# pfnet/pfrl

Hardware: AMD Instinct MI355X
Metric: env-steps/sec whole node (DQN 256 envs sharded over the GPUs) (higher is better)
Workload: dtype f32

## Files before the change

### include/pfrl_amd.h

```cpp
#ifndef PFRL_AMD_H
#define PFRL_AMD_H

#include <stdint.h>

#ifdef __cplusplus
extern "C" {
#endif

#define PFRL_TAG_ABSENT 0
#define PFRL_TAG_PY 1
#define PFRL_TAG_F32 2
#define PFRL_TAG_F64 3

#define PFRL_MAX_LEVELS 40
#define PFRL_MAX_NSTEP 16
#define PFRL_MAX_STACK 8

#define PFRL_OPT_MAX_TENSORS 24

#define PFRL_POW_CORRECTLY_ROUNDED 0
#define PFRL_POW_GLIBC 1
#define PFRL_POW_GLIBC_FMA 2
#define PFRL_ERR_ARG (-2)

// ... 241 lines not shown
                           float *g_sigma_b, int64_t out_features, int64_t in_features,
                           void *stream);

int pfrl_conv2d_nhwc_fwd(const float *x, const float *w, const float *bias, float *y, int32_t N,
                         int32_t H, int32_t W, int32_t C, int32_t Cout, int32_t R, int32_t S,
                         int32_t stride, int32_t relu, int32_t planar_out, int32_t splits,
                         void *stream);
int pfrl_conv2d_nhwc_bwd_data(const float *dy, const float *dy_mask, const float *w,
                              const float *a_prev, float *dx, int32_t N, int32_t H, int32_t W,
                              int32_t C, int32_t Cout, int32_t R, int32_t S, int32_t stride,
                              int32_t perm_p, int32_t perm_c, void *stream);
int pfrl_conv2d_nhwc_bwd_weight(const float *dy, const float *dy_mask, const float *x, float *dw_part,
                                float *db_part, int64_t dw_stride, int64_t db_stride, int32_t N,
                                int32_t H, int32_t W, int32_t C, int32_t Cout, int32_t R, int32_t S,
                                int32_t stride, int32_t splits, void *stream);
int pfrl_conv2d_u8nhwc4_fwd(const uint8_t *x, float divisor, const float *w, const float *bias,
                            float *y, int32_t N, int32_t H, int32_t W, int32_t Cout, int32_t R,
                            int32_t S, int32_t stride, int32_t relu, int32_t planar_out, void *stream);
int pfrl_conv2d_u8nhwc4_bwd_weight(const float *dy, const float *dy_mask, const uint8_t *x,
                                   float divisor, float *dw_part, float *db_part, int64_t dw_stride,
                                   int64_t db_stride, int32_t N, int32_t H, int32_t W, int32_t Cout,
                                   int32_t R, int32_t S, int32_t stride, int32_t splits, void *stream);
int pfrl_conv2d_nhwc_bwd_weight_ride(
    const float *dy, const float *dy_mask, const float *x, float *dw_part, float *db_part,
    int64_t dw_stride, int64_t db_stride, int32_t N, int32_t H, int32_t W, int32_t C, int32_t Cout,
    int32_t R, int32_t S, int32_t stride, int32_t splits, int32_t n_ride, float *const *ride_param,
    const float *const *ride_grad, float *const *ride_square_avg, float *const *ride_grad_avg,
    const int64_t *ride_numel, float lr, float alpha, float eps, float weight_decay, int centered,
    void *stream);
int pfrl_conv2d_nhwc_bwd(const float *dy, const float *dy_mask, const float *w, const float *a_prev,
                         const float *x, float *dx, float *dw_part, float *db_part, int64_t dw_stride,
                         int64_t db_stride, int32_t N, int32_t H, int32_t W, int32_t C, int32_t Cout,
                         int32_t R, int32_t S, int32_t stride, int32_t perm_p, int32_t perm_c,
                         int32_t splits, void *stream);
int pfrl_splitk_reduce(int32_t n_tasks, const float *const *host_part, float *const *host_out,
                       const float *const *host_bias, const int64_t *host_stride,
                       const int32_t *host_n, const int32_t *host_splits, const int32_t *host_ncol,
                       const int32_t *host_relu, void *stream);
int pfrl_clip_grad_norm(int32_t n_tensors, float *const *grads, const int64_t *numel, float max_norm,
                        double *partial_ws, float *out_norm_coef, void *stream);
int pfrl_splitk_group(const float *part, int64_t stride, int32_t n, int32_t splits, int32_t groups,
                      float *out, int64_t out_stride, void *stream);
int pfrl_linear_fwd(const float *x, const float *w, const float *bias, float *y, int32_t M, int32_t K,
                    int32_t N, int32_t relu, int32_t splits, void *stream);
int pfrl_linear_bwd_weight(const float *dy, const float *dy_mask, const float *x, float *dw_part,
                           float *db_part, int64_t dw_stride, int64_t db_stride, int32_t M, int32_t K,
                           int32_t N, int32_t splits, void *stream);
int pfrl_linear_small_fwd(const float *x, const float *w, const float *bias, float *y, int32_t M,
                          int32_t K, int32_t N, void *stream);
int pfrl_dqn_act_head(const float *h, const float *w, const float *bias, const int32_t *choice,
                      float *q, int64_t *greedy, int64_t *action, int32_t M, int32_t K, int32_t N,
                      void *stream);
int pfrl_qnet_plan_images(int32_t images);
int pfrl_linear_small_bwd(const float *dy, const float *x, const float *w, float *dx, float *dw,
                          float *db, int32_t M, int32_t K, int32_t N, void *stream);

int pfrl_linear_fwd_twin(const float *const *x, const float *const *x2, int32_t K1,
                         const float *const *w, const float *const *bias, float *const *y, int32_t M,
                         int32_t K, int32_t N, int32_t relu, void *stream);
int pfrl_linear_bwd_twin(const float *const *dy, const float *const *dy_mask, const float *const *w,
                         const float *const *x, const float *const *x2, int32_t K1, float *const *dx,
                         float *const *dw_part,
                         float *const *db_part, int64_t dw_stride, int64_t db_stride, int32_t M,
                         int32_t K, int32_t N, int32_t splits, void *stream);
int pfrl_linear_small_fwd_twin(const float *const *x, const float *const *w, const float *const *bias,
                               float *const *y, int32_t M, int32_t K, int32_t N, void *stream);
int pfrl_linear_small_bwd_twin(const float *const *dy, const float *const *x, const float *const *w,
                               float *const *dx, float *const *dw, float *const *db, int32_t M,
                               int32_t K, int32_t N, void *stream);
int pfrl_twin_input_grad(const float *const *dy, const float *const *dy_mask, const float *const *w,
                         int32_t ldw, int32_t col0, int32_t ncol, float *dx, int32_t M, int32_t N,
                         void *stream);

int pfrl_squashed_gaussian_fwd(const float *loc, int64_t ld_loc, const float *scale, int64_t ld_scale,
                               const float *eps, float *action, float *logp, float *neg_logp, int32_t B,
                               int32_t A, void *stream);
int pfrl_squashed_gaussian_bwd(const float *g_action, const float *g_logp, const float *action,
                               const float *eps, const float *scale, int64_t ld_scale, float *g_loc,
                               float *g_scale, int32_t B, int32_t A, void *stream);
int pfrl_squashed_head_fwd(const float *x, int64_t ldx, float clamp_lo, float clamp_hi, int32_t mode,
                           const float *eps, float *action, float *logp, float *neg_logp, int32_t B,
                           int32_t A, void *stream);
int pfrl_squashed_head_bwd(const float *g_action, const float *g_logp, const float *action,
                           const float *eps, const float *x, int64_t ldx, float clamp_lo, float clamp_hi,
                           int32_t mode, float *g_x, int32_t B, int32_t A, void *stream);
int pfrl_soft_update(int32_t n_tensors, float *const *dst, const float *const *src,
                     const int64_t *numel, double tau, void *stream);
int pfrl_adam_step(int32_t n_tensors, float *const *params, const float *const *grads,
                   float *const *exp_avg, float *const *exp_avg_sq, float *const *steps,
                   const int64_t *numel, double lr, double beta1, double beta2, double eps,
                   double weight_decay, void *ticket, void *stream);
int pfrl_adam_step_ex(int32_t n_tensors, float *const *params, const float *const *grads,
                      const int64_t *slab_stride, const int32_t *n_slabs, float *const *exp_avg,
                      float *const *exp_avg_sq, float *const *steps, float *const *soft_dst, double tau,
                      const int64_t *numel, double lr, double beta1, double beta2, double eps,
                      double weight_decay, void *ticket, void *stream);
int pfrl_sac_temperature_loss(const float *log_temperature, const float *log_prob,
                              float entropy_target, float *loss, int32_t B, void *stream);
int pfrl_sac_temperature_step(float *log_temperature, const float *log_prob, float entropy_target,
                              float *loss, float *exp_avg, float *exp_avg_sq, float *step, double lr,
                              double beta1, double beta2, double eps, double weight_decay, int32_t B,
                              void *stream);
int pfrl_sac_target_q(const float *reward, const float *discount, const float *terminal,
                      const float *next_q1, const float *next_q2, const float *next_log_prob,
                      const float *log_temperature, float temperature, float *target_q, int32_t B,
                      void *stream);
// ... 86 lines not shown
```

### pfrl_amd/_native.py

```python
import ctypes
import os
import shutil
import subprocess

_HERE = os.path.dirname(os.path.abspath(__file__))
CSRC = os.path.join(_HERE, "csrc")
LIB_DIR = os.path.join(_HERE, "lib")
LIB_PATH = os.path.join(LIB_DIR, "libpfrl_amd.so")
_LIB_OVERRIDE = os.environ.get("PFRL_AMD_LIB")
SOURCES = ["frames.hip", "replay.hip", "sumtree.hip", "rollout.hip", "optim.hip", "tdloss.hip", "bias_act.hip", "noisy.hip", "c51.hip", "dueling.hip", "qnet.hip", "actor.hip", "hostplan.hip", "philox.hip", "ppo_gaussian.hip", "trpo.hip"]
HIPCC_FLAGS = [
    "--offload-arch=gfx950", "-O3", "-std=c++17", "-fPIC",
    "-ffp-contract=off", "-fno-fast-math",
    "-mllvm", "-amdgpu-kernarg-preload-count=16",
    "-mllvm", "-amdgpu-mfma-vgpr-form",
]

MAX_LEVELS = 40
MAX_NSTEP = 16
MAX_STACK = 8


def _hipcc():
    for cand in (shutil.which("hipcc"), "/opt/rocm/bin/hipcc"):
# ... 123 lines not shown
    "pfrl_tree_update_errors_write_sample": (ctypes.c_int, "Rqppifdifdddiiqppppqpppppppppidqpp"),
    "pfrl_tree_sample": (ctypes.c_int, "Rqpppppppppidqpp"),
    "pfrl_tree_update_errors_f32": (ctypes.c_int, "Rqppifdifdddiip"),
    "pfrl_tree_update_errors_write_f32": (ctypes.c_int, "Rqppifdifdddiiqppppp"),
    "pfrl_h2d_async": (ctypes.c_int, "ppqp"),
    "pfrl_powf_host": (ctypes.c_int, "ipfpq"),
    "pfrl_powf_host_variant": (ctypes.c_int, "fq"),
    "pfrl_powf_device": (ctypes.c_int, "ipfpqp"),
    "pfrl_tree_set_priorities": (ctypes.c_int, "Rqpppip"),
    "pfrl_gae_scan": (ctypes.c_int, "qqpppppddippp"),
    "pfrl_a2c_returns": (ctypes.c_int, "qqppppddip"),
    "pfrl_adv_stats": (ctypes.c_int, "pqppp"),
    "pfrl_ppo_minibatch": (ctypes.c_int, "qpppipppppippppppp"),
    "pfrl_ppo_act_head": (ctypes.c_int, "pppppppppppiiipp"),
    "pfrl_ppo_loss": (ctypes.c_int, "pppppppiiffffppppp"),
    "pfrl_ppo_head_loss": (ctypes.c_int, "ppppppppppiiiffffppippp"),
    "pfrl_ppo_gaussian_act": (ctypes.c_int, "pppppppiip"),
    "pfrl_ppo_gaussian_loss": (ctypes.c_int, "ppppppppiiffffpppppp"),
    "pfrl_ppo_minibatch_f32act": (ctypes.c_int, "qpppippppipippppppp"),
    "pfrl_trpo_gaussian_eval": (ctypes.c_int, "pppppppiifppppp"),
    "pfrl_cg_workgroup_reach": (ctypes.c_int, []),
    "pfrl_cg_init": (ctypes.c_int, "ppppppqp"),
    "pfrl_cg_step": (ctypes.c_int, "ppppppqfp"),
    "pfrl_trpo_scale_step": (ctypes.c_int, "ppdpppqp"),
    "pfrl_params_axpy": (ctypes.c_int, "ippppfp"),
    "pfrl_rmsprop_step": (ctypes.c_int, "ipppppffffip"),
    "pfrl_rmsprop_fused_step": (ctypes.c_int, "ipffffip"),
    "pfrl_dqn_td_loss": (ctypes.c_int, "ppppppppqiiippppp"),
    "pfrl_dqn_head_td_loss": (ctypes.c_int, "ppppppppppiiiiipppppiqpppfp"),
    "pfrl_bias_relu_fwd": (ctypes.c_int, "pppqiqp"),
    "pfrl_bias_relu_bwd": (ctypes.c_int, "ppppppqiiqp"),
    "pfrl_c51_loss": (ctypes.c_int, "pppppppppiiiippppp"),
    "pfrl_dueling_softmax_fwd": (ctypes.c_int, "pppqiip"),
    "pfrl_dueling_softmax_bwd": (ctypes.c_int, "ppppqiip"),
    "pfrl_noisy_weights_fwd": (ctypes.c_int, "pppppppqqp"),
    "pfrl_noisy_weights_bwd": (ctypes.c_int, "pppppqqp"),
    "pfrl_conv2d_nhwc_fwd": (ctypes.c_int, "ppppiiiiiiiiiiip"),
    "pfrl_conv2d_nhwc_bwd_data": (ctypes.c_int, "pppppiiiiiiiiiip"),
    "pfrl_conv2d_nhwc_bwd_weight": (ctypes.c_int, "pppppqqiiiiiiiiip"),
    "pfrl_conv2d_nhwc_bwd_weight_ride": (ctypes.c_int, "pppppqqiiiiiiiiiipppppffffip"),
    "pfrl_conv2d_nhwc_bwd": (ctypes.c_int, "ppppppppqqiiiiiiiiiiip"),
    "pfrl_splitk_reduce": (ctypes.c_int, "ippppppppp"),
    "pfrl_splitk_reduce_noisy": (ctypes.c_int, "ippppppppppp"),
    "pfrl_splitk_group": (ctypes.c_int, "pqiiipqp"),
    "pfrl_clip_grad_norm": (ctypes.c_int, "ippfppp"),
    "pfrl_linear_noisy_fwd": (ctypes.c_int, "pppppppiiiiip"),
    "pfrl_linear_noisy_fwd_pair": (ctypes.c_int, "pippppppiipip"),
    "pfrl_linear_fwd": (ctypes.c_int, "ppppiiiiip"),
    "pfrl_linear_bwd_weight": (ctypes.c_int, "pppppqqiiiip"),
    "pfrl_linear_small_fwd": (ctypes.c_int, "ppppiiip"),
    "pfrl_linear_small_bwd": (ctypes.c_int, "ppppppiiip"),
    "pfrl_dqn_act_head": (ctypes.c_int, "pppppppiiip"),
    "pfrl_qnet_plan_images": (ctypes.c_int, "i"),
    "pfrl_squashed_gaussian_fwd": (ctypes.c_int, "pqpqppppiip"),
    "pfrl_squashed_gaussian_bwd": (ctypes.c_int, "pppppqppiip"),
    "pfrl_squashed_head_fwd": (ctypes.c_int, "pqffippppiip"),
    "pfrl_squashed_head_bwd": (ctypes.c_int, "pppppqffipiip"),
    "pfrl_soft_update": (ctypes.c_int, "ipppdp"),
    "pfrl_adam_step": (ctypes.c_int, "ippppppdddddpp"),
    "pfrl_adam_step_ex": (ctypes.c_int, "ippppppppdpdddddpp"),
    "pfrl_sac_temperature_loss": (ctypes.c_int, "ppfpip"),
    "pfrl_sac_temperature_step": (ctypes.c_int, "ppfppppdddddip"),
    "pfrl_sac_target_q": (ctypes.c_int, "pppppppfpip"),
    "pfrl_half_mse_fwd": (ctypes.c_int, "pppip"),
    "pfrl_half_mse_bwd": (ctypes.c_int, "ppppip"),
    "pfrl_half_mse_twin_fwd": (ctypes.c_int, "ppppip"),
    "pfrl_half_mse_twin_bwd": (ctypes.c_int, "ppppip"),
    "pfrl_linear_fwd_twin": (ctypes.c_int, "ppipppiiiip"),
    "pfrl_linear_bwd_twin": (ctypes.c_int, "pppppipppqqiiiip"),
    "pfrl_linear_small_fwd_twin": (ctypes.c_int, "ppppiiip"),
    "pfrl_linear_small_bwd_twin": (ctypes.c_int, "ppppppiiip"),
    "pfrl_twin_input_grad": (ctypes.c_int, "pppiiipiip"),
    "pfrl_sac_policy_loss_fwd": (ctypes.c_int, "ppppfppppip"),
    "pfrl_sac_policy_loss_bwd": (ctypes.c_int, "ppppfpppip"),
    "pfrl_philox_normal": (ctypes.c_int, "QQipppppip"),
    "pfrl_profile_enable": (ctypes.c_int, "i"),
    "pfrl_profile_collect": (ctypes.c_int64, "pppq"),
}

_CODES = {
    "p": ctypes.c_void_p, "q": ctypes.c_int64, "Q": ctypes.c_uint64, "i": ctypes.c_int,
    "f": ctypes.c_float, "d": ctypes.c_double,
    "T": ctypes.POINTER(TableDesc), "R": ctypes.POINTER(TreeDesc),
    "H": ctypes.POINTER(HostStoreDesc), "P": ctypes.c_void_p,
}

_lib = None


def lib():
    global _lib
    if _lib is not None:
        return _lib
    if not os.path.exists(LIB_PATH):
        raise RuntimeError(
            "pfrl_amd: %s is missing.  The device replay path has no CPU fallback; "
            "run `python -c 'import __graft_entry__ as g; g.build()'` (needs hipcc)." % LIB_PATH
        )
    L = ctypes.CDLL(_LIB_OVERRIDE or LIB_PATH)
    for name, (res, args) in EXPORTS.items():
        fn = getattr(L, name)
        fn.restype = res
        fn.argtypes = [_CODES[c] for c in args] if isinstance(args, str) else args
    _lib = L
    return L

# ... 52 lines not shown
```

### pfrl_amd/agents/dqn.py

```python
import collections
import copy
import os
from logging import getLogger

import numpy as np
import torch
import torch.nn.functional as F

from pfrl_amd import agent
from pfrl_amd.replay_buffer import (AbstractEpisodicReplayBuffer, DeviceExperienceBatch,
                                    ReplayUpdater, batch_experiences,
                                    batch_recurrent_experiences)
from pfrl_amd.utils.batch_states import batch_states
from pfrl_amd.utils.clip_l2_grad_norm import clip_l2_grad_norm_
from pfrl_amd.utils.contexts import evaluating
from pfrl_amd.utils.copy_param import synchronize_parameters
from pfrl_amd.utils.recurrent import (get_recurrent_state_at, mask_recurrent_state_at,
                                      one_step_forward, pack_and_forward,
                                      recurrent_state_as_numpy)


class _Pending:
    def __repr__(self):
        return "greedy(pending)"
# ... 98 lines not shown
        self.gamma = gamma
        self.explorer = explorer
        self.gpu = gpu
        self.target_update_interval = target_update_interval
        self.clip_delta = clip_delta
        self.phi = phi
        self.target_update_method = target_update_method
        self.soft_update_tau = soft_update_tau
        self.batch_accumulator = batch_accumulator
        assert batch_accumulator in ("mean", "sum")
        self.logger = logger
        self.batch_states = batch_states
        self.replay_updater = ReplayUpdater(
            replay_buffer=replay_buffer,
            update_func=self.update_from_episodes if self.recurrent else self.update,
            batchsize=minibatch_size,
            episodic_update=self.recurrent, episodic_update_len=episodic_update_len,
            n_times_update=n_times_update, replay_start_size=replay_start_size,
            update_interval=update_interval)
        self.minibatch_size = minibatch_size
        self.episodic_update_len = episodic_update_len
        self.replay_start_size = replay_start_size
        self.update_interval = update_interval
        self.max_grad_norm = max_grad_norm
        assert target_update_interval % update_interval == 0, \
            "target_update_interval should be a multiple of update_interval"
        self.t = 0
        self.optim_t = 0
        self._cumulative_steps = 0
        self.target_model = make_target_model_as_copy(self.model)
        self.q_record = _DeviceRecord(1000)
        self.loss_record = _DeviceRecord(100)
        self.batch_last_obs = []
        self.batch_last_action = []
        self.train_recurrent_states = None
        self.train_prev_recurrent_states = None
        self.test_recurrent_states = None
        if (self.replay_buffer.capacity is not None
                and self.replay_buffer.capacity < self.replay_updater.replay_start_size):
            raise ValueError("Replay start size cannot exceed replay buffer capacity.")
        from pfrl_amd.distributed import GradientAllReducer

        self.grad_reducer = GradientAllReducer(self.model)
        on_gpu = self.device.type == "cuda"
        self.use_graphs = on_gpu if use_graphs is None else bool(use_graphs and on_gpu)
        self.step_fused_gather = on_gpu if step_fused_gather is None else \
            bool(step_fused_gather and on_gpu)
        self.batch_target_pass = self.step_fused_gather if batch_target_pass is None else \
            bool(batch_target_pass and self.step_fused_gather)
        self.fused_td_loss = bool(fused_td_loss)
        self.step_fused_chunks = tuple(step_fused_chunks)
        self._chunks_set_by_caller = tuple(step_fused_chunks) != (0.1, 0.4)
        self._target_raw_bufs = {}
        self._single_bufs = {}
        self.range_graphs = os.environ.get("PFRL_RANGE_GRAPHS", "1") != "0"
        self.device_step = (on_gpu and self.step_fused_gather
                            and os.environ.get("PFRL_DEVICE_STEP", "1") != "0")
        self._last_actions_dev = None
        self._analytic_backward = None
        self._graphed = None
        self._last_y = None
        self._replay_stream = None
        self._fwd_event = None
        from pfrl_amd.replay_buffers.prioritized import PrioritizedReplayBuffer

        want_overlap = (self.use_graphs and isinstance(replay_buffer, PrioritizedReplayBuffer)
                        and getattr(replay_buffer, "is_device", False))
        if want_overlap if replay_overlap is None else (replay_overlap and want_overlap):
            self._replay_stream = torch.cuda.Stream(self.device)
            self._fwd_event = torch.cuda.Event()
            self._replay_stream.wait_stream(torch.cuda.current_stream(self.device))
            replay_buffer.set_replay_stream(self._replay_stream)

    @property
    def cumulative_steps(self):
        return self._cumulative_steps

    def sync_target_network(self):
        self._flush_backward()
        synchronize_parameters(src=self.model, dst=self.target_model,
                               method=self.target_update_method, tau=self.soft_update_tau)

    def update(self, experiences, errors_out=None, _gathered=None):
        self._flush_backward()
        if isinstance(experiences, DeviceExperienceBatch):
            has_weight = experiences.has_weight
        else:
            has_weight = "weight" in experiences[0][0]
        exp_batch = _gathered if _gathered is not None else batch_experiences(
            experiences, device=self.device, phi=self.phi, gamma=self.gamma,
            batch_states=self.batch_states)
        if self._replay_stream is not None and isinstance(experiences, DeviceExperienceBatch):
            if self._graphed is not None and self.use_graphs and has_weight:
                self._graphed.prefill(exp_batch, True)
            torch.cuda.current_stream(self.device).wait_event(experiences.store.ready_event)
        if has_weight and "weights" not in exp_batch:
            exp_batch["weights"] = torch.tensor([e[0]["weight"] for e in experiences],
                                                device=self.device, dtype=torch.float32)
        self._update_from_batch(exp_batch, has_weight, errors_out)

    def update_from_episodes(self, episodes, errors_out=None):
        assert errors_out is None, "Recurrent DQN does not support PrioritizedBuffer"
        episodes = sorted(episodes, key=len, reverse=True)
        exp_batch = batch_recurrent_experiences(episodes, device=self.device, phi=self.phi,
                                                gamma=self.gamma, batch_states=self.batch_states)
        self._update_from_batch(exp_batch)
# ... 35 lines not shown

    _late = None
    _in_train_step = False

    def _late_backward_ok(self):
        if self.__dict__.get("_late") is None:
            self._late = []
            self._late_enabled = os.environ.get("PFRL_LATE_BACKWARD", "1") != "0"
        return (self._late_enabled and self._in_train_step
                and not getattr(self._graphed, "split_for_allreduce", False))

    def _flush_backward(self):
        late = self.__dict__.get("_late")
        if late:
            pending = list(late)
            del late[:]
            for replay_rest in pending:
                replay_rest()

    def _graphed_step(self, exp_batch, want_errors, deferred=None, after_forward=None, late=None):
        if self._graphed is None:
            from pfrl_amd.agents.graphed_update import GraphedUpdate

            self._graphed = GraphedUpdate(self)
            self._graphed.pipeline = self._replay_stream is not None
        try:
            loss, delta, y = self._graphed.run(exp_batch, want_errors, after_forward, late)
        except Exception as e:
            if self._graphed.graphs:
                raise
            self.logger.warning("HIP-graph capture of the update failed (%s); running eagerly", e)
            self.use_graphs = False
            loss, delta = self._compute_loss(exp_batch, want_errors=want_errors)
            self.loss_record.extend(loss)
            self.optimizer.zero_grad()
            loss.backward()
            self.grad_reducer.all_reduce()
            if self.max_grad_norm is not None:
                clip_l2_grad_norm_(self.model.parameters(), self.max_grad_norm)
            self.optimizer.step()
            return loss, delta
        if deferred is not None:
            deferred.append((loss, y))
        else:
            self.loss_record.extend(loss.clone())
            self.q_record.extend(y.clone())
        return loss, delta

    def _target_is_deterministic(self):
        from pfrl_amd.nn.noisy_linear import FactorizedNoisyLinear

        return not any(isinstance(m, (FactorizedNoisyLinear, torch.nn.Dropout))
                       for m in self.target_model.modules())

    def _precompute_target_raw(self, next_states):
        with torch.no_grad():
            av = self.target_model(next_states)
        if hasattr(av, "q_dist"):
            self._target_z_values = av.z_values
            return av.q_dist
        return av.q_values

    def _action_value(self, model, states, recurrent_state):
        if self.recurrent:
            return pack_and_forward(model, states, recurrent_state)[0]
        return model(states)

    def _target_next_action_value(self, exp_batch):
        raw = exp_batch.get("target_next_raw")
        if raw is None:
            return self._action_value(self.target_model, exp_batch["next_state"],
                                      exp_batch.get("next_recurrent_state"))
        if raw.ndim == 3:
            from pfrl_amd.action_value import DistributionalDiscreteActionValue

            return DistributionalDiscreteActionValue(raw, self._target_z_values)
        from pfrl_amd.action_value import DiscreteActionValue

        return DiscreteActionValue(raw)

    def _compute_target_values(self, exp_batch):
        target_next_qout = self._target_next_action_value(exp_batch)
        next_q_max = target_next_qout.max
        return (exp_batch["reward"]
                + exp_batch["discount"] * (1.0 - exp_batch["is_state_terminal"]) * next_q_max)

    def _compute_y_and_t(self, exp_batch):
        batch_size = exp_batch["reward"].shape[0]
        qout = self._action_value(self.model, exp_batch["state"], exp_batch.get("recurrent_state"))
        batch_q = torch.reshape(qout.evaluate_actions(exp_batch["action"]), (batch_size, 1))
        with torch.no_grad():
            batch_q_target = torch.reshape(self._compute_target_values(exp_batch), (batch_size, 1))
        return batch_q, batch_q_target


    def _fused_td_loss_applicable(self):
        cls = type(self)
        if not (self.fused_td_loss and self.device.type == "cuda" and not self.recurrent
                and cls._fused_td_double is not None
                and cls._compute_y_and_t is DQN._compute_y_and_t
                and cls._compute_loss is DQN._compute_loss):
            return False
        if cls._fused_td_double:
            from pfrl_amd.agents.double_dqn import DoubleDQN

            return cls._compute_target_values is DoubleDQN._compute_target_values
# ... 328 lines not shown

    def _observe_range_fused(self, lo, hi, batch_obs, batch_reward, batch_done, batch_reset):
        plan = self._plan_and_fetch_range(lo, hi, batch_obs, batch_reward, batch_done, batch_reset)
        self._run_range_updates(lo, hi, plan)

    def _plan_and_fetch_range(self, lo, hi, batch_obs, batch_reward, batch_done, batch_reset):
        rbuf = self.replay_buffer
        up = self.replay_updater
        t0 = self.t
        plan_env, plan_seqs = [], []
        native = None
        if self.device_step and self.__dict__.get("_obs_cols") is not None:
            from pfrl_amd.agents import _dqn_device_step

            native = _dqn_device_step.plan_range(self, lo, hi, batch_obs)
        if native is not None:
            plan_env, slots_dev, U = native
        elif self._batched_append_ok(lo, hi, batch_obs):
            prev = self._last_obs_batch
            lens, heads = rbuf.append_batch_n1(
                prev.refs[lo:hi], prev.min_seq[lo:hi],
                np.asarray(self.batch_last_action[lo:hi], dtype=np.int64),
                np.asarray(batch_reward[lo:hi], dtype=np.float64),
                batch_obs.refs[lo:hi], batch_obs.min_seq[lo:hi],
                np.asarray(batch_done[lo:hi], dtype=np.uint8))
            for i in range(lo, hi):
                if batch_reset[i] or batch_done[i]:
                    self.batch_last_obs[i] = None
                    self.batch_last_action[i] = None
                j = i - lo
                if (lens[j] >= up.replay_start_size
                        and (t0 + j + 1) % up.update_interval == 0):
                    for _ in range(up.n_times_update):
                        plan_env.append(i)
                        plan_seqs.append(rbuf.lookahead_sample_at(lens[j], heads[j], up.batchsize))
        else:
            for i in range(lo, hi):
                self._append_transition(i, batch_obs, batch_reward, batch_done, batch_reset)
                if (len(rbuf) >= up.replay_start_size
                        and (t0 + (i - lo) + 1) % up.update_interval == 0):
                    for _ in range(up.n_times_update):
                        plan_env.append(i)
                        plan_seqs.append(rbuf.lookahead_sample(up.batchsize))
        if native is not None:
            big = rbuf.store.fetch_many_slots(slots_dev, U, up.batchsize, self.phi,
                                              self.gamma) if U else None
        else:
            big = rbuf.fetch_many(plan_seqs, self.phi, self.gamma) if plan_seqs else None
        if big is not None and self.batch_target_pass and self._target_is_deterministic():
            tui = self.target_update_interval
            if (t0 + (hi - lo)) // tui == t0 // tui:
                ns = big["next_state"]
                U, B = ns.shape[0], ns.shape[1]
                raw = self._precompute_target_raw(ns.view((U * B,) + tuple(ns.shape[2:])))
                key = (U, B, getattr(rbuf.store, "many_parity", 0)) + tuple(raw.shape[1:])
                buf = self._target_raw_bufs.get(key)
                if buf is None:
                    buf = self._target_raw_bufs[key] = torch.empty(
                        (U, B) + tuple(raw.shape[1:]), dtype=raw.dtype, device=raw.device)
                buf.view(raw.shape).copy_(raw)
                big["target_next_raw"] = buf
        return plan_env, big, t0

    def _run_range_updates(self, lo, hi, plan):
        plan_env, big, t0 = plan
        if big is not None and self._range_as_one_graph(t0, hi - lo):
            try:
                losses, ys = self._graphed.run_range(big)
            except Exception as e:
                if self._graphed.graphs:
                    raise
                self.logger.warning("HIP-graph capture of an env range failed (%s); updating "
                                    "one minibatch at a time", e)
                self.range_graphs = False
            else:
                self.t += hi - lo
                self._cumulative_steps += hi - lo
                self.loss_record.extend(losses.clone())
                self.q_record.extend(ys.clone())
                self.optim_t += len(plan_env)
                return
        p = 0
        deferred = [] if self.use_graphs else None
        staged = (big is not None and self.use_graphs and self.range_graphs
                  and self._graphed is not None and self._graphed.range_capturable())
        if staged:
            deferred = None
        for i in range(lo, hi):
            self.t += 1
            self._cumulative_steps += 1
            if self.t % self.target_update_interval == 0:
                self.sync_target_network()
            while p < len(plan_env) and plan_env[p] == i:
                mb = {k: v[p] for k, v in big.items()}
                if staged:
                    mb = self._stage_minibatch(mb)
                self._update_from_batch(mb, deferred=deferred)
                p += 1
        if deferred and self.use_graphs:
            if len({id(l) for l, _ in deferred}) == len(deferred):
                self.loss_record.extend(torch.stack([l.reshape(()) for l, _ in deferred]))
                self.q_record.extend(torch.cat([y.reshape(-1) for _, y in deferred]))
            else:
                for l, y in deferred:
                    self.loss_record.extend(l.clone())
                    self.q_record.extend(y.clone())

    def _stage_minibatch(self, mb):
# ... 81 lines not shown
```

### pfrl_amd/csrc/qnet.hip

```cpp
#include <type_traits>

#include "common.h"
#include "rms_update.h"

namespace {

typedef float f32x4 __attribute__((ext_vector_type(4)));

constexpr int KC = 32;
#ifndef PFRL_LDR
#define PFRL_LDR (KC + 4)
#endif
constexpr int LDR = PFRL_LDR;

struct FastDiv {
    uint32_t m = 1, s1 = 0, s2 = 0;
};
static FastDiv fast_div(uint32_t d) {
    FastDiv f;
    uint32_t l = 0;
    while ((1ull << l) < d) ++l;
    f.m = (uint32_t)((((1ull << l) - d) << 32) / d + 1);
    f.s1 = l < 1 ? l : 1;
    f.s2 = l < 1 ? 0 : l - 1;
// ... 2355 lines not shown

extern "C" int pfrl_splitk_group(const float *part, int64_t stride, int32_t n, int32_t splits,
                                 int32_t groups, float *out, int64_t out_stride, void *stream) {
    PFRL_CHECK_ARG(part && out && n >= 1 && splits >= 1 && groups >= 1 && groups <= splits &&
                       stride % 4 == 0 && out_stride % 4 == 0 && out_stride >= n,
                   "pfrl_splitk_group: bad arguments (strides % 4, groups <= splits)");
    const int per = (splits + groups - 1) / groups;
    PFRL_CHECK_ARG((long long)per * (groups - 1) < splits, "pfrl_splitk_group: an empty group");
    hipLaunchKernelGGL(k_splitk_group, dim3((n + RED_CHUNK - 1) / RED_CHUNK, groups), dim3(256), 0,
                       (hipStream_t)stream, part, (long long)stride, n, splits, per, out,
                       (long long)out_stride);
    PFRL_LAUNCH_CHECK();
}

#define SMALL_DISPATCH(N, CALL)                                            \
    switch (N) {                                                           \
        case 1: CALL(1); break;   case 2: CALL(2); break;   case 3: CALL(3); break;   \
        case 4: CALL(4); break;   case 5: CALL(5); break;   case 6: CALL(6); break;   \
        case 7: CALL(7); break;   case 8: CALL(8); break;   case 9: CALL(9); break;   \
        case 10: CALL(10); break; case 11: CALL(11); break; case 12: CALL(12); break; \
        case 13: CALL(13); break; case 14: CALL(14); break; case 15: CALL(15); break; \
        default: CALL(16); break;                                          \
    }

static int small_fwd_launch(const SmallFwdArgs &a, int twins, int32_t M, int32_t K, int32_t N,
                            void *stream) {
    PFRL_CHECK_ARG(N >= 1 && N <= SMALL_N && M >= 1 && K >= 1, "pfrl_linear_small_fwd: N <= 16");
#define CALL_FWD(NN)                                                                             \
    hipLaunchKernelGGL(k_linear_small_fwd<NN>, dim3(M, twins), dim3(256), 0, (hipStream_t)stream, a, K)
    SMALL_DISPATCH(N, CALL_FWD)
#undef CALL_FWD
    PFRL_LAUNCH_CHECK();
}

extern "C" int pfrl_linear_small_fwd(const float *x, const float *w, const float *bias, float *y,
                                     int32_t M, int32_t K, int32_t N, void *stream) {
    SmallFwdArgs a{{x, nullptr}, {w, nullptr}, {bias, nullptr}, {y, nullptr}};
    return small_fwd_launch(a, 1, M, K, N, stream);
}

extern "C" int pfrl_dqn_act_head(const float *h, const float *w, const float *bias, const int32_t *choice,
                                 float *q, int64_t *greedy, int64_t *action, int32_t M, int32_t K,
                                 int32_t N, void *stream) {
    PFRL_CHECK_ARG(N >= 1 && N <= SMALL_N && M >= 1 && K >= 1, "pfrl_dqn_act_head: 1 <= N <= 16");
    PFRL_CHECK_ARG(h && w && (q || greedy || action), "pfrl_dqn_act_head: null argument");
#define CALL_ACT(NN)                                                                             \
    hipLaunchKernelGGL(k_dqn_act_head<NN>, dim3(M), dim3(256), 0, (hipStream_t)stream, h, w, bias, \
                       choice, q, greedy, action, K)
    SMALL_DISPATCH(N, CALL_ACT)
#undef CALL_ACT
    PFRL_LAUNCH_CHECK();
}

static int small_bwd_launch(const SmallBwdArgs &a, int twins, bool want_dx, bool want_dw, int32_t M,
                            int32_t K, int32_t N, void *stream) {
    const int NP = N <= SMALL_N ? N : (N + 7) / 8 * 8;
    PFRL_CHECK_ARG(N >= 1 && N <= SMALL_BWD_N && M >= 1 && K >= 1 && (size_t)M * NP * 4 <= 40 * 1024,
                   "pfrl_linear_small_bwd: N <= 64, M * (N rounded up to 8 above 16) <= 10240");
    PFRL_CHECK_ARG(want_dw || want_dx, "pfrl_linear_small_bwd: nothing to compute");
    const int n_dw = want_dw ? (K + 31) / 32 : 0;
    const dim3 grid(n_dw + (want_dx ? ((K + 255) / 256) * ((M + 7) / 8) : 0), twins);
#define CALL_BWD(NN)                                                                              \
    hipLaunchKernelGGL(k_linear_small_bwd<NN>, grid, dim3(256), (size_t)M * NP * sizeof(float),  \
                       (hipStream_t)stream, a, M, K, n_dw, N)
    if (N <= SMALL_N) {
        SMALL_DISPATCH(N, CALL_BWD)
    } else if (N <= 24) CALL_BWD(24);
    else if (N <= 32) CALL_BWD(32);
    else if (N <= 40) CALL_BWD(40);
    else if (N <= 48) CALL_BWD(48);
    else if (N <= 56) CALL_BWD(56);
    else CALL_BWD(64);
#undef CALL_BWD
    PFRL_LAUNCH_CHECK();
}

namespace {

template <int NT>
__global__ __launch_bounds__(256) void k_linear_narrow_bwd(
    const float *__restrict__ dy, const float *__restrict__ x, const float *__restrict__ w,
    float *__restrict__ dx, float *__restrict__ dw, float *__restrict__ db, int M, int K, int NR, int n_dw) {
    constexpr int NP = 16 * NT, LD = NP + 1;
    extern __shared__ float sdy[];
    __shared__ float comb[2][NT][64][4];
    const int tid = threadIdx.x, wave = __builtin_amdgcn_readfirstlane(tid >> 6), lane = tid & 63;
    const int r16 = lane & 15, q = lane >> 4;
    const int M16 = (M + 15) / 16 * 16, KT = (K + 15) / 16;
    constexpr int DYL = 64;
    float dv[DYL];
    const int ndl = (M * NR + 255) / 256;
#pragma unroll
    for (int g8 = 0; g8 < DYL / 8; ++g8)
        if (8 * g8 < ndl) {
#pragma unroll
            for (int u = 8 * g8; u < 8 * g8 + 8; ++u) dv[u] = dy[min(tid + 256 * u, M * NR - 1)];
        }
    const bool dw_role = (int)blockIdx.x < n_dw;
    constexpr int BMAX = 32;
    float b[BMAX];
    int tile, mh = 0, Mh = 0, mt_lo = 0, mt_hi = 0;
    bool ones = false, idle = false;
    if (dw_role) {
        tile = blockIdx.x * 2 + (wave >> 1);
        mh = wave & 1;
        Mh = M16 / 2;
// ... 417 lines not shown
```

### pfrl_amd/nn/mfma_trunk.py

```python
import contextlib
import ctypes
import os

import torch
import torch.nn as nn

from pfrl_amd import _native
from pfrl_amd._native import check

_ENABLED = os.environ.get("PFRL_MFMA_TRUNK", "1") != "0"
_MAX_BATCH = int(os.environ.get("PFRL_MFMA_TRUNK_MAX_BATCH", "0"))
SMALL_LINEAR_MAX_OUT = 16


_raw_stream = getattr(torch._C, "_cuda_getCurrentRawStream", None)


def _stream():
    if _raw_stream is not None:
        return ctypes.c_void_p(_raw_stream(torch.cuda.current_device()))
    return ctypes.c_void_p(torch.cuda.current_stream().cuda_stream)


def _p(t):
# ... 464 lines not shown
                grads[2 * i], grads[2 * i + 1] = None, None
            if i > 0 and _fused_bwd_ok(N, sp.H, sp.W, sp.C, sp.ST,
                                       (sp.R // sp.ST) * (sp.S // sp.ST)):
                dx = torch.empty((N, sp.H, sp.W, sp.C), dtype=torch.float32, device=dev)
                check(lib.pfrl_conv2d_nhwc_bwd(_p(dy), None, _p(w), _p(below), _p(below), _p(dx), _p(pw),
                                               _p(pb), st, st, N, sp.H, sp.W, sp.C, sp.Cout, sp.R, sp.S,
                                               sp.ST, 0, 0, splits, _stream()), "conv2d_nhwc_bwd")
                dy = dx
                continue
            ra = RIDE_ALONG.ride_arrays([(p_, g_) for p_, g_, _ in ride]) if (ride and i == 0) else None
            if ra is not None:
                from pfrl_amd.optimizers import GradSource

                check(lib.pfrl_conv2d_nhwc_bwd_weight_ride(
                    _p(dy), None, _p(below), _p(pw), _p(pb), st, st, N, sp.H, sp.W, sp.C, sp.Cout, sp.R,
                    sp.S, sp.ST, splits, *ra, _stream()), "conv2d_nhwc_bwd_weight_ride")
                for p_, g_, slot in ride:
                    OPT_SOURCES[p_.data_ptr()] = GradSource.done()
                    grads[slot] = None
                continue
            u8d = getattr(ctx, "u8_divisor", None)
            if i == 0 and u8d is not None:
                check(lib.pfrl_conv2d_u8nhwc4_bwd_weight(_p(dy), None, _p(below), u8d, _p(pw), _p(pb),
                                                         st, st, N, sp.H, sp.W, sp.Cout, sp.R, sp.S,
                                                         sp.ST, splits, _stream()),
                      "conv2d_u8nhwc4_bwd_weight")
                continue
            check(lib.pfrl_conv2d_nhwc_bwd_weight(_p(dy), None, _p(below), _p(pw), _p(pb), st, st, N,
                                                  sp.H, sp.W, sp.C, sp.Cout, sp.R, sp.S, sp.ST, splits,
                                                  _stream()), "conv2d_nhwc_bwd_weight")
            if i > 0:
                dx = torch.empty((N, sp.H, sp.W, sp.C), dtype=torch.float32, device=dev)
                check(lib.pfrl_conv2d_nhwc_bwd_data(_p(dy), None, _p(w), _p(below), _p(dx), N, sp.H,
                                                    sp.W, sp.C, sp.Cout, sp.R, sp.S, sp.ST, 0, 0,
                                                    _stream()), "conv2d_nhwc_bwd_data")
                dy = dx
        if OPT_SOURCES is None and _DEFERRED_FOLDS and len(tasks) + len(_DEFERRED_FOLDS) <= 12:
            tasks += _DEFERRED_FOLDS
            del _DEFERRED_FOLDS[:]
        if tasks:
            _reduce(tasks)
        return (None, None) + tuple(grads)


def trunk_forward(x, specs, convs, linear):
    params = []
    for c in convs:
        params += [c.weight, c.bias]
    if linear is not None:
        params += [linear.weight, linear.bias]
    return _Trunk.apply(x, specs, *params)


class _SmallLinear(torch.autograd.Function):

    @staticmethod
    def forward(ctx, x, w, b):
        M, K = x.shape
        Nout = w.shape[0]
        x = x.contiguous()
        y = torch.empty((M, Nout), dtype=torch.float32, device=x.device)
        check(_native.lib().pfrl_linear_small_fwd(_p(x), _p(w), _p(b), _p(y), M, K, Nout, _stream()),
              "linear_small_fwd")
        ctx.save_for_backward(x, w)
        ctx.has_bias = b is not None
        return y

    @staticmethod
    def backward(ctx, dy):
        x, w = ctx.saved_tensors
        M, K = x.shape
        Nout = w.shape[0]
        dy = dy.contiguous()
        dx = torch.empty_like(x) if ctx.needs_input_grad[0] else None
        if not ctx.needs_input_grad[1]:
            if dx is None:
                return None, None, None
            check(_native.lib().pfrl_linear_small_bwd(_p(dy), _p(x), _p(w), _p(dx), None, None, M, K,
                                                      Nout, _stream()), "linear_small_bwd")
            return dx, None, None
        dw = torch.empty_like(w)
        db = torch.empty(Nout, dtype=torch.float32, device=x.device) if ctx.has_bias else None
        check(_native.lib().pfrl_linear_small_bwd(_p(dy), _p(x), _p(w), _p(dx), _p(dw), _p(db), M, K,
                                                  Nout, _stream()), "linear_small_bwd")
        return dx, dw, db


def small_linear_supported(layer, x):
    return (_ENABLED and isinstance(layer, nn.Linear) and x.is_cuda and x.dim() == 2
            and x.dtype == torch.float32 and layer.out_features <= SMALL_LINEAR_MAX_OUT
            and layer.weight.dtype == torch.float32 and layer.weight.is_contiguous()
            and x.shape[0] * layer.out_features <= 10240 and x.shape[0] <= 4096
            and _native.available())


def small_linear(x, layer):
    return _SmallLinear.apply(x, layer.weight, layer.bias)


class _SmallLinearSlot(nn.Linear):

    def __init__(self, linear):
        nn.Module.__init__(self)
        self.__dict__.update({k: v for k, v in linear.__dict__.items()
                              if k not in ("_parameters", "_buffers", "_modules")})
        self._parameters = linear._parameters
# ... 67 lines not shown
```

### pfrl_amd/utils/copy_param.py

```python
import torch


def copy_param(target_link, source_link):
    target_link.load_state_dict(source_link.state_dict())


def _same_dense_layout(dst, src):
    return (dst.stride() == src.stride()
            and (dst.is_contiguous()
                 or (dst.dim() == 4 and dst.is_contiguous(memory_format=torch.channels_last))))


def soft_copy_params(pairs, tau):
    fdst, fsrc = [], []
    for target_link, source_link in pairs:
        tgt = target_link.state_dict()
        for name, src in source_link.state_dict().items():
            dst = tgt[name]
            if dst.dtype in (torch.int32, torch.int64):
                dst.copy_(src)
            else:
                assert dst.shape == src.shape, name
                fdst.append(dst)
                fsrc.append(src)
    if not fdst:
        return
    rest = []
    if fdst[0].is_cuda:
        import ctypes

        from pfrl_amd import _native

        fused = [(d, s) for d, s in zip(fdst, fsrc)
                 if d.is_cuda and s.is_cuda and d.device == s.device and d.dtype == torch.float32
                 and s.dtype == torch.float32 and _same_dense_layout(d, s)]
        fused_ids = {id(d) for d, _ in fused}
        rest = [(d, s) for d, s in zip(fdst, fsrc) if id(d) not in fused_ids]
        if fused:
            n = len(fused)
            Dp = (ctypes.c_void_p * n)(*[d.data_ptr() for d, _ in fused])
            Sp = (ctypes.c_void_p * n)(*[s.data_ptr() for _, s in fused])
            L = (ctypes.c_int64 * n)(*[d.numel() for d, _ in fused])
            stream = ctypes.c_void_p(torch.cuda.current_stream(fused[0][0].device).cuda_stream)
            _native.check(_native.lib().pfrl_soft_update(n, Dp, Sp, L, float(tau), stream),
                          "soft_update")
    else:
        rest = list(zip(fdst, fsrc))
    for dst, src in rest:
        dst.mul_(1 - tau)
        dst.add_(tau * src)


def soft_copy_param(target_link, source_link, tau):
    soft_copy_params([(target_link, source_link)], tau)


def copy_grad(target_link, source_link):
    for tp, sp in zip(target_link.parameters(), source_link.parameters()):
        assert tp.shape == sp.shape
        tp.grad = None if sp.grad is None else sp.grad.clone()


def synchronize_parameters(src, dst, method, tau=None):
    if method == "hard":
        copy_param(dst, src)
    elif method == "soft":
# ... 4 lines not shown
```

Before: 42260.

## Add native single-call Nature-DQN target Q inference pass

```diff
diff --git a/include/pfrl_amd.h b/include/pfrl_amd.h
--- a/include/pfrl_amd.h
+++ b/include/pfrl_amd.h
@@ -317,6 +317,13 @@
                       float *q, int64_t *greedy, int64_t *action, int32_t M, int32_t K, int32_t N,
                       void *stream);
 int pfrl_qnet_plan_images(int32_t images);
+int pfrl_nature_q_infer(const void *x, int32_t x_u8, float divisor, float *x_f32, const float *w1,
+                        const float *b1, const float *w2, const float *b2, const float *w3,
+                        const float *b3, const float *wf, const float *bf, float *wf_nhwc,
+                        int32_t refresh_wf_nhwc, const float *wq, const float *bq, float *a1, float *a2,
+                        float *a3, float *h, float *h_part, int32_t fc_splits, float *q,
+                        int64_t q_row_offset, int32_t rows, int32_t hidden, int32_t n_actions,
+                        void *stream);
 int pfrl_linear_small_bwd(const float *dy, const float *x, const float *w, float *dx, float *dw,
                           float *db, int32_t M, int32_t K, int32_t N, void *stream);
 
diff --git a/pfrl_amd/_native.py b/pfrl_amd/_native.py
--- a/pfrl_amd/_native.py
+++ b/pfrl_amd/_native.py
@@ -199,6 +199,7 @@
     "pfrl_linear_small_bwd": (ctypes.c_int, "ppppppiiip"),
     "pfrl_dqn_act_head": (ctypes.c_int, "pppppppiiip"),
     "pfrl_qnet_plan_images": (ctypes.c_int, "i"),
+    "pfrl_nature_q_infer": (ctypes.c_int, "pifppppppppppipppppppipqiiip"),
     "pfrl_squashed_gaussian_fwd": (ctypes.c_int, "pqpqppppiip"),
     "pfrl_squashed_gaussian_bwd": (ctypes.c_int, "pppppqppiip"),
     "pfrl_squashed_head_fwd": (ctypes.c_int, "pqffippppiip"),
diff --git a/pfrl_amd/agents/dqn.py b/pfrl_amd/agents/dqn.py
--- a/pfrl_amd/agents/dqn.py
+++ b/pfrl_amd/agents/dqn.py
@@ -174,6 +174,8 @@
         self.step_fused_chunks = tuple(step_fused_chunks)
         self._chunks_set_by_caller = tuple(step_fused_chunks) != (0.1, 0.4)
         self._target_raw_bufs = {}
+        self.native_target_pass = os.environ.get("PFRL_NATIVE_TARGET_PASS", "1") != "0"
+        self._native_target = None
         self._single_bufs = {}
         self.range_graphs = os.environ.get("PFRL_RANGE_GRAPHS", "1") != "0"
         self.device_step = (on_gpu and self.step_fused_gather
@@ -315,6 +317,17 @@
 
         return not any(isinstance(m, (FactorizedNoisyLinear, torch.nn.Dropout))
                        for m in self.target_model.modules())
+
+    def _native_target_parts(self, next_states):
+        if not self.native_target_pass or self.device.type != "cuda" or self.recurrent \
+                or type(self)._precompute_target_raw is not DQN._precompute_target_raw \
+                or not torch.is_tensor(next_states) or self.target_model.training:
+            return None
+        from pfrl_amd.nn.mfma_trunk import NatureQPass
+
+        if self._native_target is None:
+            self._native_target = NatureQPass()
+        return NatureQPass.admits(self.target_model, next_states)
 
     def _precompute_target_raw(self, next_states):
         with torch.no_grad():
@@ -749,8 +762,21 @@
             if (t0 + (hi - lo)) // tui == t0 // tui:
                 ns = big["next_state"]
                 U, B = ns.shape[0], ns.shape[1]
-                raw = self._precompute_target_raw(ns.view((U * B,) + tuple(ns.shape[2:])))
-                key = (U, B, getattr(rbuf.store, "many_parity", 0)) + tuple(raw.shape[1:])
+                x = ns.view((U * B,) + tuple(ns.shape[2:]))
+                parity = getattr(rbuf.store, "many_parity", 0)
+                parts = self._native_target_parts(x)
+                if parts is not None:
+                    A = parts[1].out_features
+                    key = (U, B, parity, A)
+                    buf = self._target_raw_bufs.get(key)
+                    if buf is None:
+                        buf = self._target_raw_bufs[key] = torch.empty(
+                            (U, B, A), dtype=torch.float32, device=x.device)
+                    self._native_target.run(parts, x, buf.view(U * B, A))
+                    big["target_next_raw"] = buf
+                    return plan_env, big, t0
+                raw = self._precompute_target_raw(x)
+                key = (U, B, parity) + tuple(raw.shape[1:])
                 buf = self._target_raw_bufs.get(key)
                 if buf is None:
                     buf = self._target_raw_bufs[key] = torch.empty(
diff --git a/pfrl_amd/csrc/qnet.hip b/pfrl_amd/csrc/qnet.hip
--- a/pfrl_amd/csrc/qnet.hip
+++ b/pfrl_amd/csrc/qnet.hip
@@ -2431,6 +2431,93 @@
     PFRL_LAUNCH_CHECK();
 }
 
+
+__global__ __launch_bounds__(256) void k_fc_weight_nhwc(const float *__restrict__ w, float *__restrict__ wp,
+                                                        int C, int P, long long n) {
+    const long long i = (long long)blockIdx.x * 256 + threadIdx.x;
+    if (i >= n) return;
+    const int K = C * P;
+    const long long f = i / K;
+    const int k = (int)(i - f * K), p = k / C, c = k - p * C;
+    wp[i] = w[f * K + (long long)c * P + p];
+}
+
+__global__ __launch_bounds__(256) void k_u8_phi(const uint8_t *__restrict__ x, float *__restrict__ y, float d,
+                                                long long n) {
+    const long long i = (long long)blockIdx.x * 256 + threadIdx.x;
+    if (i < n) y[i] = __fdiv_rn((float)x[i], d);
+}
+
+extern "C" int pfrl_nature_q_infer(const void *x, int32_t x_u8, float divisor, float *x_f32,
+                                   const float *w1, const float *b1, const float *w2, const float *b2,
+                                   const float *w3, const float *b3, const float *wf, const float *bf,
+                                   float *wf_nhwc, int32_t refresh_wf_nhwc, const float *wq,
+                                   const float *bq, float *a1, float *a2, float *a3, float *h,
+                                   float *h_part, int32_t fc_splits, float *q, int64_t q_row_offset,
+                                   int32_t rows, int32_t hidden, int32_t n_actions, void *stream) {
+    constexpr int C3 = 64, P3 = 49, KF = C3 * P3;
+    PFRL_CHECK_ARG(x && w1 && b1 && w2 && b2 && w3 && b3 && wf && bf && a1 && a2 && a3 && h,
+                   "pfrl_nature_q_infer: null pointer");
+    PFRL_CHECK_ARG(rows >= 1 && hidden >= 32 && hidden % 32 == 0 && fc_splits >= 1 && q_row_offset >= 0,
+                   "pfrl_nature_q_infer: rows >= 1, hidden % 32 == 0, splits >= 1, row offset >= 0");
+    PFRL_CHECK_ARG(fc_splits == 1 || h_part != nullptr, "pfrl_nature_q_infer: split-K needs h_part");
+    PFRL_CHECK_ARG(wq == nullptr || (q != nullptr && n_actions >= 1 && n_actions <= SMALL_N),
+                   "pfrl_nature_q_infer: the narrow head needs q and 1 <= n_actions <= 16");
+    hipStream_t st = (hipStream_t)stream;
+    int rc;
+    if (x_u8) {
+        FwdArgs a;
+        a.M = (long long)rows * (D1_O * D1_O);
+        a.K = 256;
+        a.cps = a.K / KC;
+        const int prog = fwd_program(a, 32, 1, plan_rows(a.M, rows));
+        if (prog == 3 || prog == 4 || prog == 8) {
+            rc = pfrl_conv2d_u8nhwc4_fwd(static_cast<const uint8_t *>(x), divisor, w1, b1, a1, rows, D1_HW,
+                                         D1_HW, 32, 8, 8, 4, 1, 0, stream);
+        } else {
+            PFRL_CHECK_ARG(x_f32 != nullptr && divisor > 0.f,
+                           "pfrl_nature_q_infer: a u8 batch this small needs the x_f32 scratch");
+            const long long n = (long long)rows * D1_HW * D1_HW * 4;
+            hipLaunchKernelGGL(k_u8_phi, dim3((unsigned)((n + 255) / 256)), dim3(256), 0, st,
+                               static_cast<const uint8_t *>(x), x_f32, divisor, n);
+            rc = pfrl_conv2d_nhwc_fwd(x_f32, w1, b1, a1, rows, D1_HW, D1_HW, 4, 32, 8, 8, 4, 1, 0, 1, stream);
+        }
+    } else {
+        rc = pfrl_conv2d_nhwc_fwd(static_cast<const float *>(x), w1, b1, a1, rows, D1_HW, D1_HW, 4, 32, 8, 8,
+                                  4, 1, 0, 1, stream);
+    }
+    if (rc != 0) return rc;
+    rc = pfrl_conv2d_nhwc_fwd(a1, w2, b2, a2, rows, 20, 20, 32, 64, 4, 4, 2, 1, 0, 1, stream);
+    if (rc != 0) return rc;
+    const bool nhwc_fc = wf_nhwc != nullptr;
+    rc = pfrl_conv2d_nhwc_fwd(a2, w3, b3, a3, rows, 9, 9, 64, C3, 3, 3, 1, 1, nhwc_fc ? 0 : 1, 1, stream);
+    if (rc != 0) return rc;
+    if (nhwc_fc && refresh_wf_nhwc) {
+        const long long n = (long long)hidden * KF;
+        hipLaunchKernelGGL(k_fc_weight_nhwc, dim3((unsigned)((n + 255) / 256)), dim3(256), 0, st, wf, wf_nhwc,
+                           C3, P3, n);
+    }
+    const float *wh = nhwc_fc ? wf_nhwc : wf;
+    if (fc_splits == 1) {
+        rc = pfrl_conv2d_nhwc_fwd(a3, wh, bf, h, rows, 1, 1, KF, hidden, 1, 1, 1, 1, 0, 1, stream);
+        if (rc != 0) return rc;
+    } else {
+        rc = pfrl_conv2d_nhwc_fwd(a3, wh, nullptr, h_part, rows, 1, 1, KF, hidden, 1, 1, 1, 0, 0, fc_splits,
+                                  stream);
+        if (rc != 0) return rc;
+        const float *part = h_part, *bias = bf;
+        const int64_t stride = (int64_t)rows * hidden;
+        const int32_t n = rows * hidden, ncol = hidden, relu = 1;
+        PFRL_CHECK_ARG(stride < (1ll << 31), "pfrl_nature_q_infer: rows * hidden < 2^31");
+        rc = pfrl_splitk_reduce(1, &part, &h, &bias, &stride, &n, &fc_splits, &ncol, &relu, stream);
+        if (rc != 0) return rc;
+    }
+    if (wq != nullptr)
+        return pfrl_linear_small_fwd(h, wq, bq, q + (size_t)q_row_offset * n_actions, rows, hidden, n_actions,
+                                     stream);
+    PFRL_LAUNCH_CHECK();
+}
+
 static int small_bwd_launch(const SmallBwdArgs &a, int twins, bool want_dx, bool want_dw, int32_t M,
                             int32_t K, int32_t N, void *stream) {
     const int NP = N <= SMALL_N ? N : (N + 7) / 8 * 8;
diff --git a/pfrl_amd/nn/mfma_trunk.py b/pfrl_amd/nn/mfma_trunk.py
--- a/pfrl_amd/nn/mfma_trunk.py
+++ b/pfrl_amd/nn/mfma_trunk.py
@@ -540,6 +540,130 @@
     return _Trunk.apply(x, specs, *params)
 
 
+_NATURE_CONVS = ((4, 32, 8, 4), (32, 64, 4, 2), (64, 64, 3, 1))
+
+
+def nature_q_parts(model):
+    from pfrl_amd.nn import atari_cnn
+    from pfrl_amd.q_functions import DiscreteActionValueHead
+
+    if not (type(model) is nn.Sequential and len(model) == 3):
+        return None
+    trunk, head, tail = list(model._modules.values())
+    if not (isinstance(trunk, atari_cnn._AtariCNN) and atari_cnn._is_relu(trunk.activation)
+            and type(head) in (nn.Linear, _SmallLinearSlot) and type(tail) is DiscreteActionValueHead):
+        return None
+    convs, fc = list(trunk.layers), trunk.output
+    if len(convs) != len(_NATURE_CONVS) or type(fc) is not nn.Linear or fc.bias is None:
+        return None
+    for conv, (C, Co, k, st) in zip(convs, _NATURE_CONVS):
+        if not (type(conv) is nn.Conv2d and conv.bias is not None and conv.groups == 1
+                and (conv.in_channels, conv.out_channels) == (C, Co) and conv.kernel_size == (k, k)
+                and conv.stride == (st, st) and conv.padding == (0, 0) and conv.dilation == (1, 1)
+                and conv.padding_mode == "zeros"):
+            return None
+    if not (fc.in_features == 3136 and fc.out_features % 32 == 0 and head.bias is not None
+            and head.in_features == fc.out_features and 1 <= head.out_features <= SMALL_LINEAR_MAX_OUT):
+        return None
+    return trunk, head
+
+
+class _F32Shape:
+
+    is_cuda, dtype, requires_grad = True, torch.float32, False
+
+    def __init__(self, shape):
+        self.shape = shape
+
+    def dim(self):
+        return len(self.shape)
+
+
+class NatureQPass:
+
+    def __init__(self):
+        self._scratch = {}
+        self._wp = None
+        self._wp_key = None
+
+    @staticmethod
+    def admits(model, x):
+        from pfrl_amd.ops import U8Pixels, u8_division_exact
+
+        parts = nature_q_parts(model)
+        if parts is None or tuple(x.shape[1:]) != (4, 84, 84) or x.shape[0] < 1:
+            return None
+        trunk, head = parts
+        if isinstance(x, U8Pixels):
+            d = x.data
+            if not (_ENABLED and _U8_FIRST and _native.available() and d.is_cuda
+                    and d.dtype == torch.uint8 and d.is_contiguous() and d.data_ptr() % 16 == 0
+                    and u8_division_exact(x.divisor)):
+                return None
+            probe = _F32Shape(x.shape)
+        else:
+            if not x.is_contiguous(memory_format=torch.channels_last) or x.data_ptr() % 16:
+                return None
+            probe = x
+        if plan_for(list(trunk.layers), trunk.output, probe) is None:
+            return None
+        ok = all(p.is_cuda and p.dtype == torch.float32 for p in (head.weight, head.bias))
+        return parts if ok and head.weight.is_contiguous() else None
+
+    def _buffers(self, rows, F, splits, dev, small_u8):
+        key = (rows, F, splits, small_u8, dev)
+        s = self._scratch.get(key)
+        if s is None:
+            if len(self._scratch) > 8:
+                self._scratch.clear()
+            e = lambda *shape: torch.empty(shape, dtype=torch.float32, device=dev)
+            s = self._scratch[key] = (e(rows, 20 * 20 * 32), e(rows, 9 * 9 * 64), e(rows, 3136),
+                                      e(rows, F), e(splits, rows, F) if splits > 1 else None,
+                                      e(rows, 84 * 84 * 4) if small_u8 else None)
+        return s
+
+    def _nhwc_weight(self, wf):
+        from pfrl_amd.utils import copy_param
+
+        key = (wf.data_ptr(), wf._version, copy_param.WRITE_EPOCH, tuple(wf.shape), wf.device)
+        fresh = key != self._wp_key
+        if fresh:
+            if self._wp is None or self._wp.shape != wf.shape or self._wp.device != wf.device:
+                self._wp = torch.empty_like(wf)
+            self._wp_key = key
+        return self._wp, fresh
+
+    def run(self, parts, x, out, row_offset=0):
+        from pfrl_amd.ops import U8Pixels
+
+        trunk, head = parts
+        rows = x.shape[0]
+        u8 = isinstance(x, U8Pixels)
+        data = x.data if u8 else x
+        F, A = trunk.output.out_features, head.out_features
+        assert (out.dtype == torch.float32 and out.is_contiguous() and out.dim() == 2
+                and out.shape[1] == A and 0 <= row_offset and row_offset + rows <= out.shape[0]
+                and out.device == data.device)
+        planned = max(rows, _PLAN_BATCH)
+        splits = _fwd_splits(rows, F, 3136)
+        a1, a2, a3, h, part, x32 = self._buffers(rows, F, splits, data.device, u8 and rows < 64)
+        wf = trunk.output.weight
+        wp, fresh = self._nhwc_weight(wf) if 0 < _NHWC_FC_MIN_BATCH <= planned else (None, False)
+        native_head = small_linear_supported(head, h)
+        c = trunk.layers
+        check(_native.lib().pfrl_nature_q_infer(
+            _p(data), int(u8), x.divisor if u8 else 1.0, _p(x32),
+            _p(c[0].weight), _p(c[0].bias), _p(c[1].weight), _p(c[1].bias), _p(c[2].weight),
+            _p(c[2].bias), _p(wf), _p(trunk.output.bias), _p(wp), int(fresh),
+            _p(head.weight) if native_head else None, _p(head.bias) if native_head else None,
+            _p(a1), _p(a2), _p(a3), _p(h), _p(part), splits, _p(out), row_offset, rows, F, A,
+            _stream()), "nature_q_infer")
+        if not native_head:
+            with torch.no_grad():
+                torch.addmm(head.bias, h, head.weight.t(), out=out[row_offset:row_offset + rows])
+        return out
+
+
 class _SmallLinear(torch.autograd.Function):
 
     @staticmethod
diff --git a/pfrl_amd/utils/copy_param.py b/pfrl_amd/utils/copy_param.py
--- a/pfrl_amd/utils/copy_param.py
+++ b/pfrl_amd/utils/copy_param.py
@@ -1,7 +1,11 @@
 import torch
+
+WRITE_EPOCH = 0
 
 
 def copy_param(target_link, source_link):
+    global WRITE_EPOCH
+    WRITE_EPOCH += 1
     target_link.load_state_dict(source_link.state_dict())
 
 
@@ -12,6 +16,8 @@
 
 
 def soft_copy_params(pairs, tau):
+    global WRITE_EPOCH
+    WRITE_EPOCH += 1
     fdst, fsrc = [], []
     for target_link, source_link in pairs:
         tgt = target_link.state_dict()
```

Result: no change. 42150 (-0.2%).
